# QWERTY6191/projected-lmc

Measured on AMD Instinct MI355X. Metric: MLL+grad iters/sec, n=8192 16-task LMC, higher is better.
Workload: dtype f32; 1 GPU; C3: ProjectedGPModel+ProjectedLMCmll exact training step (PLMC_fast), n=8192 d=8 p=16 q=8 Matern-5/2 fp32; latents sharded q/N per GPU; n_points=8192, n_dim=8, n_tasks=16, n_latents=8, parallelism=latent-shard x1

## Files before the change

### include/plmc.h

```cpp
#ifndef PLMC_H
#define PLMC_H

#include <stddef.h>
#include <stdint.h>

#ifdef __cplusplus
extern "C" {
#endif

enum { PLMC_RBF = 0, PLMC_MATERN12 = 1, PLMC_MATERN32 = 2, PLMC_MATERN52 = 3, PLMC_SPLINE = 4 };

int         plmc_version(void);
int         plmc_block(void);
int64_t     plmc_pad(int64_t n);
int         plmc_max_dim(void);
const char *plmc_last_error(void);
int64_t     plmc_vd_blocks_for(int64_t n_pad, int64_t lda, int elem_bytes);
int64_t     plmc_vd_blocks(int64_t n_pad, int64_t lda);
int64_t     plmc_vd_blocks_keep(int64_t n_pad, int64_t lda);
int64_t     plmc_split_scales_offset(int64_t n_pad, int64_t lda);
int64_t     plmc_grad_scratch_bytes_for(int64_t n_pad, int q, int elem_bytes);
int64_t     plmc_grad_scratch_bytes(int64_t n_pad, int q);
int64_t     plmc_grad_partials_bytes(int64_t n_pad, int q);

// ... 35 lines not shown
int plmc_potrs_aug_f64(double *A, int64_t n_pad, int64_t lda, int naug, int64_t wcol0, int64_t strideA, double *Vd, int q, void *stream);
int plmc_potrs_aug_kept_f32(float *A, int64_t n_pad, int64_t lda, int naug, int64_t wcol0, int64_t strideA, float *Vd, int q,
                            const float *eig_lo, void *stream);
int plmc_potrs_aug_kept_f64(double *A, int64_t n_pad, int64_t lda, int naug, int64_t wcol0, int64_t strideA, double *Vd, int q,
                            const double *eig_lo, void *stream);

int plmc_extract_col_f32(const float *A, int64_t n_pad, int64_t lda, int64_t strideA, int c,
                         float *z, double *quad, int q, void *stream);
int plmc_extract_col_f64(const double *A, int64_t n_pad, int64_t lda, int64_t strideA, int c,
                         double *z, double *quad, int q, void *stream);

int plmc_wt_matvec_f32(const float *W, int64_t n_pad, int64_t ldw, int64_t strideW, const float *z,
                       float *alpha, int q, void *stream);
int plmc_wt_matvec_f64(const double *W, int64_t n_pad, int64_t ldw, int64_t strideW, const double *z,
                       double *alpha, int q, void *stream);

int plmc_gemm_tn_f32(int mode, int M, int N, int K, const float *A, int64_t lda, int64_t strideA, const float *B,
                     int64_t ldb, int64_t strideB, float *C, int64_t ldc, int64_t strideC, int batch, void *stream);
int plmc_gemm_tn_f64(int mode, int M, int N, int K, const double *A, int64_t lda, int64_t strideA, const double *B,
                     int64_t ldb, int64_t strideB, double *C, int64_t ldc, int64_t strideC, int batch, void *stream);
#define PLMC_TRI_A_LOWER 1
#define PLMC_TRI_B_LOWER 2
#define PLMC_TRI_A_UPPER 4
#define PLMC_TRI_C_LOWER 8
#define PLMC_TRI_C_ZERO 16
int plmc_gemm_tn_tri_f32(int mode, int tri, int M, int N, int K, const float *A, int64_t lda, int64_t strideA, const float *B,
                         int64_t ldb, int64_t strideB, float *C, int64_t ldc, int64_t strideC, int batch, void *stream);
int plmc_gemm_tn_tri_f64(int mode, int tri, int M, int N, int K, const double *A, int64_t lda, int64_t strideA, const double *B,
                         int64_t ldb, int64_t strideB, double *C, int64_t ldc, int64_t strideC, int batch, void *stream);

// ... 147 lines not shown
```

### projected-lmc_amd/csrc/potrf.hip

```cpp
#include <stdlib.h>
#include "api_common.hpp"
#include "covariance.hpp"
#include "diag_block.hpp"
#include "bf3_engine.hpp"
#include "chain_engine.hpp"
#include "vd_layout.hpp"
#include "../../include/plmc.h"

namespace plmc {

template <typename T> constexpr int CHAIN_BURST = sizeof(T) == 8 ? 4 : 8;

template <typename T> struct ColMap {
  int u0, nU, Taug, w0, nW;
  int64_t n_pad;
  T *W;
  int64_t ldw, strideW;
};

template <typename T, int NT, bool BURSTED = false>
__global__ __launch_bounds__(NTHREADS, TILE_MIN_WAVES<T>) void k_panel(T *A, int64_t lda, int64_t strideA, int r, ColMap<T> cm,
                                                     const T *__restrict__ Vd, int64_t strideV) {
  __builtin_amdgcn_s_setprio(3);
  __shared__ __align__(16) T smem[tile_smem_elems<T>()];
// ... 596 lines not shown
    for (int u = 0; u < U; ++u)
#pragma unroll
      for (int e = 0; e < EPV; ++e) s[e] += (double)v[u][e] * (double)zz[u];
  }
#pragma unroll
  for (int e = 0; e < EPV; ++e) red[rg][cl + e] = s[e];
  __syncthreads();
  if (threadIdx.x < CW) {
    double t = 0.0;
#pragma unroll
    for (int g = 0; g < NRG; ++g) t += red[g][threadIdx.x];
    alpha[(int64_t)lat * n_pad + colw + threadIdx.x] = (T)t;
  }
}

template <typename T>
__global__ __launch_bounds__(WTMV_NT) void k_w_diag(const T *__restrict__ W, int64_t n_pad, int64_t ldw, int64_t strideW,
                                                    T *__restrict__ kd) {
  using vec_t = typename Traits<T>::vec_t;
  constexpr int EPV = Traits<T>::EPV;
  constexpr int LPR = 128 / EPV;
  constexpr int NRG = WTMV_NT / LPR;
  __shared__ double red[NRG][NB];
  const int lat = blockIdx.y;
  const int cl = (threadIdx.x % LPR) * EPV, rg = threadIdx.x / LPR;
  const int64_t col0 = (int64_t)blockIdx.x * NB;
  const T *Wl = W + (int64_t)lat * strideW + col0 + cl;
  double s[EPV];
#pragma unroll
  for (int e = 0; e < EPV; ++e) s[e] = 0.0;
// ... 23 lines not shown
}

template <typename T, class S>
struct Sweep {
  static constexpr bool bf3 = !std::is_void<S>::value;
  static_assert(!bf3 || sizeof(T) == 4, "split schemes stand in for fp32 products");
  static constexpr double nb = NB, nb3 = nb * nb * nb, esz = sizeof(T);

  T *A;
  int64_t n_pad, lda, strideA, naug_pad, wcol0;
  int q, m, Taug;
  bool with_inverse, keep;
  const float *eig_lo = nullptr;
  double *logdet = nullptr;
  int *info = nullptr;
  T *Vd, *Wg, *Vg2[2], *Ph, *Pbulk;
  unsigned short *Pl[2], *Praw, *VgP2[2], *Wk, *Uk;
  float *scl;
  int64_t strideV, pl_lat, sc_lat, uk_step;
  T *WA;
  const Knobs &kn;
  double hthr;
  unsigned bulk_lds;
  int grp, ng, chain_pool;
  hipStream_t st, C = nullptr, H = nullptr;
  hipEvent_t e_entry = nullptr, e_v = nullptr, e_gh = nullptr, e_p = nullptr, e_hd = nullptr, e_tail = nullptr, e_doneC = nullptr,
             e_doneH = nullptr, e_prev = nullptr, e_sc = nullptr;

  Sweep(T *A_, int64_t n_pad_, int64_t lda_, int naug, int64_t wcol0_, int64_t strideA_, T *Vd_, int q_, bool with_inverse_, bool keep_,
        int grp_, unsigned bulk_lds_, hipStream_t st_)
// ... 168 lines not shown
      if (!WA) return;
      const int g0 = G0(gi), G = G0(gi + 1) - g0;
      hipLaunchKernelGGL((k_wtri_planes<S>), dim3(G * (G + 1) / 2, q), dim3(NTHREADS), 0, s, (const float *)WA, lda, strideA, g0, (const float *)scl,
                         sc_lat, Wk, pl_lat, n_pad);
    }
  }
  void raw_planes0(hipStream_t s, const ColMap<T> &cm) {
    if constexpr (bf3) {
      const int nt = cm.nU + cm.Taug + cm.nW;
      if (nt > 0)
        hipLaunchKernelGGL((k_raw_planes<S>), dim3(nt, G0(1), q), dim3(NTHREADS), 0, s, (const float *)A, lda, strideA, 0, cm, Praw, pl_lat, wcol0,
                           (const float *)scl, sc_lat);
    }
  }

  bool bind_streams() {
    if (!kn.serial) bind_sweep_ctx(st, 8);
    C = kn.serial ? nullptr : side_stream();
    H = kn.serial ? nullptr : (kn.bulk_streams == 1 ? st : side_stream(1));
    hipEvent_t *const ev[] = {&e_entry, &e_v, &e_gh, &e_p, &e_hd, &e_tail, &e_doneC, &e_doneH, &e_prev};
    bool la = C && H && ng > 2;
    for (int i = 0; i < 9; ++i) la = (*ev[i] = sync_event(i)) && la;
    e_sc = sync_event(12);
    return la;
  }

  int inputs(const AssembleJob *job) {
    if (job) {
      const int rc = assemble_rows(*job, (int)sizeof(T), A, lda, strideA, q, 0, m, st);
      if (rc != 0) return rc;
// ... 9 lines not shown
    raw_planes0(st, cm_buf(G0(1), m - G0(1), Taug, 0, 0));
    for (int gi = 0; gi < ng; ++gi) {
      const int g0 = G0(gi), g1 = G0(gi + 1), g2 = G0(gi + 2);
      chain(gi, st);
      vtrans(gi, st);
      wtri_planes(gi, st);
      if (bf3) {
        gpanel(g0, g1 - g0, cm_buf(g1, g2 - g1, 0, 0, 0), gi & 1, st, 1);
        gpanel(g0, g1 - g0, cm_buf(g2, m - g2, Taug, 0, g0), gi & 1, st, 0);
        update(g1, m - g1, g0, g1 - 1, cm_buf(g1, m - g1, Taug, 0, g1), st, PK_TRAIL, g2, g2, false, g2);
        update(g1, g2 - g1, g0, g1 - 1, cm_buf(g1, g2 - g1, 0, 0, 0), st, PK_TRAIL_HEAD, 0, 0, true);
      } else {
        gpanel(g0, g1 - g0, cm_buf(g1, m - g1, Taug, 0, g0), gi & 1, st, 0);
        update(g1, m - g1, g0, g1 - 1, cm_buf(g1, m - g1, Taug, 0, g1), st, PK_TRAIL);
      }
    }
    return finish(st);
  }

  int lookahead(const AssembleJob *job) {
    const bool fused = job && e_sc;
    if (fused) {
      const int rc = assemble_rows(*job, (int)sizeof(T), A, lda, strideA, q, 0, G0(1), st, G0(1));
      if (rc != 0) return rc;
      scan(st, 0, (int64_t)G0(1) * NB, 0, SCAN_PARTS / 2);
    } else {
      const int rc = inputs(job);
      if (rc != 0) return rc;
    }
    (void)hipEventRecord(e_entry, st);
// ... 16 lines not shown
      (void)hipEventRecord(e_v, C);
      if (gi > 0 || bf3) (void)hipStreamWaitEvent(C, e_hd, 0);
      gpanel(g0, G, cm_buf(g1, g2 - g1, 0, 0, 0), gi & 1, C, 1);
      (void)hipEventRecord(e_gh, C);
      if (gi > 0) (void)hipStreamWaitEvent(C, e_tail, 0);
      update(g1, g2 - g1, g0, g1 - 1, cm_buf(g1, g2 - g1, 0, 0, 0), C, PK_TRAIL_HEAD, 0, 0, true);

      (void)hipStreamWaitEvent(H, e_v, 0);
      wtri_planes(gi, H);
      gpanel(g0, G, cm_buf(g2, m - g2, Taug, 0, g0), gi & 1, H, 0);
      (void)hipEventRecord(e_p, H);
      (void)hipStreamWaitEvent(H, e_gh, 0);
      if (gi > 0) (void)hipStreamWaitEvent(H, e_tail, 0);
      update(g1, g2 - g1, g0, g1 - 1, cm_buf(g2, m - g2, Taug, 0, g1), H, PK_TRAIL_HEAD, 0, 0, false, g2);
      (void)hipEventRecord(e_hd, H);

      (void)hipStreamWaitEvent(st, e_p, 0);
      (void)hipStreamWaitEvent(st, e_gh, 0);
      update(g2, m - g2, g0, g1 - 1, cm_buf(g2, m - g2, Taug, 0, g1), st, PK_TRAIL);
      (void)hipEventRecord(e_tail, st);
    }
    const int rc_fin = finish(C);
    (void)hipEventRecord(e_doneC, C);
    (void)hipEventRecord(e_doneH, H);
    (void)hipStreamWaitEvent(st, e_doneC, 0);
    (void)hipStreamWaitEvent(st, e_doneH, 0);
    (void)hipEventRecord(e_prev, st);
    return rc_fin;
  }
};

template <typename T, class S>
int potrf_impl(T *A, int64_t n_pad, int64_t lda, int naug, int64_t strideA, T *Vd, double *logdet, int *info,
               int with_inverse_arg, int q, const float *eig_lo, void *stream, const AssembleJob *job = nullptr) {
  PLMC_REQUIRE((with_inverse_arg & 2) == 0, "with_inverse bit 1 (K^-1 accumulated in the sweep) is gone: use plmc_kinv_grad_* behind the sweep");
  const bool with_inverse = (with_inverse_arg & 1) != 0;
  const bool keep = !std::is_void<S>::value && (with_inverse_arg & 4) != 0 && with_inverse;
  PLMC_REQUIRE(A && Vd && logdet && info, "null pointer");
  PLMC_REQUIRE(n_pad > 0 && n_pad % NB == 0 && lda % NB == 0 && lda >= n_pad, "n_pad/lda must be multiples of NB");
  const int64_t naug_pad = plmc_pad(naug);
  PLMC_REQUIRE(naug >= 0 && n_pad + naug_pad + (with_inverse ? n_pad : 0) <= lda,
               "lda too small for naug (+ the n_pad columns of the inverse factor)");
  PLMC_REQUIRE(q > 0 && aligned16(A) && aligned16(Vd), "bad q or unaligned buffer");
  const Knobs &kn = knobs();
  const int grp = (!keep && kn.grp > 0 && kn.grp < GMAX) ? kn.grp : GMAX;
  const unsigned bulk_lds = (unsigned)(kn.bulk_lds >= 0 ? kn.bulk_lds : (q == 1 ? 20000 : (q == 2 ? 16000 : 0)));
  Sweep<T, S> sw(A, n_pad, lda, naug, n_pad + naug_pad, strideA, Vd, q, with_inverse, keep, grp, bulk_lds, (hipStream_t)stream);
  sw.eig_lo = eig_lo;
  sw.logdet = logdet;
  sw.info = info;
  const double npd = (double)n_pad;
  ProfScope whole(PK_SWEEP, sw.st, q * (with_inverse ? 2.0 : 1.0) * npd * npd * npd / 3.0, 0.0);
  sw.clear();
  return sw.bind_streams() ? sw.lookahead(job) : sw.one_stream(job);
}

bool vd_w_planes(const float *Vd, int64_t n_pad, int64_t lda, const unsigned short **wk, int64_t *wk_lat_stride, const float **w_scale,
                 int64_t *w_scale_lat_stride) {
  const VdLayout L(n_pad, lda, 4, false);
  if (L.wk < 0) return false;
  *wk = L.at<const unsigned short>(Vd, L.wk);
  *wk_lat_stride = L.stride_u16();
  *w_scale = L.at<const float>(Vd, L.scl) + SC_SW;
  *w_scale_lat_stride = L.stride_f32();
  return true;
// ... 85 lines not shown
  PLMC_REQUIRE(n_pad > 0 && n_pad % NB == 0 && q > 0 && aligned16(W), "n_pad must be a multiple of NB");
  ProfScope ps(PK_WTMV, (hipStream_t)stream, q * (double)n_pad * n_pad, q * ((double)n_pad * n_pad / 2) * sizeof(T));
  hipLaunchKernelGGL(k_w_diag<T>, dim3((unsigned)(n_pad / NB), q), dim3(WTMV_NT), 0, (hipStream_t)stream, W, n_pad, ldw, strideW,
                     kinv_diag);
  return launch_status(__func__);
}

}

extern "C" {
int64_t plmc_vd_blocks_for(int64_t n_pad, int64_t lda, int elem_bytes) { return plmc::VdLayout(n_pad, lda, elem_bytes, false).blocks; }
int64_t plmc_vd_blocks(int64_t n_pad, int64_t lda) { return plmc_vd_blocks_for(n_pad, lda, 4); }
int64_t plmc_vd_blocks_keep(int64_t n_pad, int64_t lda) { return plmc::VdLayout(n_pad, lda, 4, true).blocks; }
int64_t plmc_split_scales_offset(int64_t n_pad, int64_t lda) { return plmc::VdLayout(n_pad, lda, 4, false).scl * plmc::NB * plmc::NB; }
static int potrf_f32_any(float *A, int64_t n_pad, int64_t lda, int naug, int64_t strideA, float *Vd, double *logdet, int *info,
                         int with_inverse, int q, const float *eig_lo, void *stream, const plmc::AssembleJob *job = nullptr) {
  const int split = plmc::knobs().split;
  if (split == 0) return plmc::potrf_impl<float, void>(A, n_pad, lda, naug, strideA, Vd, logdet, info, with_inverse, q, nullptr, stream, job);
  if (split == 2 && eig_lo)
    return plmc::potrf_impl<float, plmc::SplitH2>(A, n_pad, lda, naug, strideA, Vd, logdet, info, with_inverse, q, eig_lo, stream, job);
  return plmc::potrf_impl<float, plmc::SplitB3>(A, n_pad, lda, naug, strideA, Vd, logdet, info, with_inverse, q, nullptr, stream, job);
}
int plmc_factorize_ex_f32(int kind, const float *X, int n, int d, const float *ell, const float *oscale, const float *noise, float *A,
                          int64_t n_pad, int64_t lda, int naug, int64_t strideA, float *Vd, double *logdet, int *info, int with_inverse, int q,
                          const float *eig_lo, void *stream) {
  PLMC_REQUIRE(n_pad == plmc_pad(n), "n_pad must be plmc_pad(n)");
  const plmc::AssembleJob job{kind, n, d, X, ell, oscale, noise};
  return potrf_f32_any(A, n_pad, lda, naug, strideA, Vd, logdet, info, with_inverse, q, eig_lo, stream, &job);
}
int plmc_factorize_ex_f64(int kind, const double *X, int n, int d, const double *ell, const double *oscale, const double *noise, double *A,
                          int64_t n_pad, int64_t lda, int naug, int64_t strideA, double *Vd, double *logdet, int *info, int with_inverse, int q,
                          const double *eig_lo, void *stream) {
  (void)eig_lo;
  PLMC_REQUIRE(n_pad == plmc_pad(n), "n_pad must be plmc_pad(n)");
  const plmc::AssembleJob job{kind, n, d, X, ell, oscale, noise};
  return plmc::potrf_impl<double, void>(A, n_pad, lda, naug, strideA, Vd, logdet, info, with_inverse, q, nullptr, stream, &job);
}
// ... 38 lines not shown
  return potrf_f32_any(A, n_pad, lda, naug, strideA, Vd, logdet, info, with_inverse, q, nullptr, stream);
}
int plmc_potrf_f64(double *A, int64_t n_pad, int64_t lda, int naug, int64_t strideA, double *Vd, double *logdet,
                   int *info, int with_inverse, int q, void *stream) {
  return plmc::potrf_impl<double, void>(A, n_pad, lda, naug, strideA, Vd, logdet, info, with_inverse, q, nullptr, stream);
}
int plmc_potrf_ex_f32(float *A, int64_t n_pad, int64_t lda, int naug, int64_t strideA, float *Vd, double *logdet,
                      int *info, int with_inverse, int q, const float *eig_lo, void *stream) {
  return potrf_f32_any(A, n_pad, lda, naug, strideA, Vd, logdet, info, with_inverse, q, eig_lo, stream);
}
int plmc_potrf_ex_f64(double *A, int64_t n_pad, int64_t lda, int naug, int64_t strideA, double *Vd, double *logdet,
                      int *info, int with_inverse, int q, const double *eig_lo, void *stream) {
  (void)eig_lo;
  return plmc::potrf_impl<double, void>(A, n_pad, lda, naug, strideA, Vd, logdet, info, with_inverse, q, nullptr, stream);
}
int plmc_potrs_aug_f32(float *A, int64_t n_pad, int64_t lda, int naug, int64_t wcol0, int64_t strideA, float *Vd, int q, void *stream) {
  return plmc::potrs_aug_at<float>(A, n_pad, lda, naug, wcol0, strideA, Vd, q, stream);
}
int plmc_potrs_aug_f64(double *A, int64_t n_pad, int64_t lda, int naug, int64_t wcol0, int64_t strideA, double *Vd, int q, void *stream) {
  return plmc::potrs_aug_at<double>(A, n_pad, lda, naug, wcol0, strideA, Vd, q, stream);
}
int plmc_potrs_aug_kept_f32(float *A, int64_t n_pad, int64_t lda, int naug, int64_t wcol0, int64_t strideA, float *Vd, int q, const float *eig_lo,
                            void *stream) {
  const int split = plmc::knobs().split;
  if (split == 0) return plmc::potrs_aug_at<float>(A, n_pad, lda, naug, wcol0, strideA, Vd, q, stream);
  if (split == 2 && eig_lo) return plmc::potrs_aug_kept<plmc::SplitH2>(A, n_pad, lda, naug, wcol0, strideA, Vd, q, stream);
  return plmc::potrs_aug_kept<plmc::SplitB3>(A, n_pad, lda, naug, wcol0, strideA, Vd, q, stream);
}
int plmc_potrs_aug_kept_f64(double *A, int64_t n_pad, int64_t lda, int naug, int64_t wcol0, int64_t strideA, double *Vd, int q, const double *eig_lo,
                            void *stream) {
// ... 27 lines not shown
```

### projected-lmc_amd/projectedlmc/_engine.py

```python
import math
import os

import torch

from . import _hip
from . import settings
from ._pivot import PivotCheck, deferred_pivot_checks, walk

LOG2PI = math.log(2.0 * math.pi)


class Workspace:

    def __init__(self, n, q, naug, dtype, device, with_inverse=True, keep_planes=False, ncomp=1, sm=False):
        L = _hip.lib()
        self.n, self.q, self.naug, self.dtype, self.device = n, q, naug, dtype, device
        self.ncomp = ncomp
        self.with_inverse = bool(with_inverse)
        self.keep_planes = bool(keep_planes) and self.with_inverse and dtype == torch.float32
        self.NB = L.cdll.plmc_block()
        self.n_pad = int(L.cdll.plmc_pad(n))
        self.naug_pad = int(L.cdll.plmc_pad(naug)) if naug > 0 else 0
        self.wcol0 = self.n_pad + self.naug_pad
        self.lda = self.wcol0 + (self.n_pad if with_inverse else 0)
# ... 2 lines not shown
        self.strideA = self.n_pad * self.lda
        esz = torch.empty((), dtype=dtype).element_size()
        vd_blocks = L.cdll.plmc_vd_blocks_keep(self.n_pad, self.lda) if self.keep_planes else L.cdll.plmc_vd_blocks_for(self.n_pad, self.lda, esz)
        self.Vd = torch.empty(q, int(vd_blocks), self.NB, self.NB, dtype=dtype, device=device)
        self.m = self.n_pad // self.NB
        self.A = torch.empty(q, self.n_pad, self.lda, dtype=dtype, device=device)
        self.logdet = torch.empty(q, dtype=torch.float64, device=device)
        self.quad = torch.empty(q, dtype=torch.float64, device=device)
        self.info = torch.empty(q, dtype=torch.int32, device=device)
        self.z = torch.empty(q, self.n_pad, dtype=dtype, device=device)
        self.W = self.alpha = self.partials = None
        if with_inverse:
            self.W = self.A[:, :, self.wcol0:self.wcol0 + self.n_pad]
            self.ldw, self.strideW = self.lda, self.strideA
            self.alpha = torch.empty(q, self.n_pad, dtype=dtype, device=device)
            nbytes = int(L.cdll.plmc_sm_grad_partials_bytes(self.n_pad, q, ncomp, esz) if sm
                         else L.cdll.plmc_grad_partials_bytes(self.n_pad, q * ncomp))
            self.partials = torch.empty(nbytes // 8, dtype=torch.float64, device=device)


_ws_cache = {}


def _release(ws):
    pending = getattr(ws, "pending", None)
    if pending is not None:
        torch.cuda.current_stream(ws.device).wait_event(pending)
        ws.pending = None


# ... 31 lines not shown

def free_workspaces():
    _drop_all()


def _contig(t, dtype=None):
    if t is None:
        return None
    t = t.detach()
    if dtype is not None and t.dtype != dtype:
        t = t.to(dtype)
    return t.contiguous()


_SM = {"plmc_assemble": "plmc_assemble_sm", "plmc_assemble_cross": "plmc_assemble_cross_sm",
       "plmc_factorize_ex": "plmc_factorize_sm_ex", "plmc_kinv_grad_vd": "plmc_kinv_grad_sm_vd"}
_ADD = {"plmc_assemble": "plmc_assemble_add", "plmc_assemble_cross": "plmc_assemble_cross_add",
        "plmc_factorize_ex": "plmc_factorize_add_ex", "plmc_kinv_grad_vd": "plmc_kinv_grad_add_vd"}


def is_sm(ell):
    return ell.dim() == 4


def n_components(ell):
    return ell.shape[2] if ell.dim() == 4 else (ell.shape[1] if ell.dim() == 3 else 1)


def kind_code(kind):
    return None if kind == "sm" else _hip.KIND[kind]


def grad_table_width(ell):
# ... 23 lines not shown
            means.record_stream(stream)
        L.call(_SM[base], dt, *head[1:], ell.shape[2], _hip.ptr(scales), _hip.ptr(means), *tail)
    elif ell.dim() == 3:
        L.call(_ADD[base], dt, *head, ell.shape[1], _hip.ptr(ell), *tail)
    else:
        L.call(base, dt, *head, _hip.ptr(ell), *tail)


def _split_grad_table(g, ell_shape, os_shape):
    ne = 1
    for s_ in ell_shape[1:]:
        ne *= s_
    return g[:, :ne].reshape(ell_shape), g[:, ne], (None if os_shape is None else g[:, ne + 1:].reshape(os_shape))


def factorize(kind, X, ell, oscale, noise, rhs, ws, Xs=None):
    L = _hip.lib()
    dt, dev = ws.dtype, ws.device
    st = _hip.stream_ptr(dev)
    k = kind_code(kind)
    q, n, d = ws.q, ws.n, X.shape[1]
    fused = os.environ.get("PLMC_FUSED_ASSEMBLE", "1") != "0"
    if not fused:
        _kernel_call(L, "plmc_assemble", dt, (k, _hip.ptr(X), n, d), ell, (_hip.ptr(oscale), _hip.ptr(noise),
                     _hip.ptr(ws.A), ws.lda, ws.strideA, q, st))
    nrhs = 0 if rhs is None else rhs.shape[1]
    if ws.naug_pad > 0:
        L.call("plmc_write_rhs", dt, _hip.ptr(rhs), nrhs, n, _hip.ptr(ws.A), ws.lda, ws.strideA, 0, ws.naug_pad, q, st)
    if Xs is not None:
        _kernel_call(L, "plmc_assemble_cross", dt, (k, _hip.ptr(X), n, _hip.ptr(Xs), Xs.shape[0], d), ell,
                     (_hip.ptr(oscale), _hip.ptr(ws.A), ws.lda, ws.strideA, ws.n_pad + nrhs, ws.n_pad, q, st))
    flags = (1 | (4 if ws.keep_planes else 0)) if ws.with_inverse else 0
    if fused:
        _kernel_call(L, "plmc_factorize_ex", dt, (k, _hip.ptr(X), n, d), ell, (_hip.ptr(oscale), _hip.ptr(noise), _hip.ptr(ws.A), ws.n_pad,
                     ws.lda, ws.naug, ws.strideA, _hip.ptr(ws.Vd), _hip.ptr(ws.logdet), _hip.ptr(ws.info), flags, q, _hip.ptr(noise), st))
    else:
        L.call("plmc_potrf_ex", dt, _hip.ptr(ws.A), ws.n_pad, ws.lda, ws.naug, ws.strideA, _hip.ptr(ws.Vd),
               _hip.ptr(ws.logdet), _hip.ptr(ws.info), flags, q, _hip.ptr(noise), st)


def factorize_checked(kind, X, ell, oscale, noise, rhs, ws, Xs=None):
    factorize(kind, X, ell, oscale, noise, rhs, ws, Xs)
    if not settings.check_cholesky.on():
        return 0.0
    check = PivotCheck.eager(ws)
    if not check.failed():
        return 0.0

    def attempt(jit):
        factorize(kind, X, ell, oscale, noise + jit, rhs, ws, Xs)
        return PivotCheck.eager(ws), None

    return walk(ws.dtype, check, attempt)[0]


class ExactLatentLogProb(torch.autograd.Function):

    @staticmethod
    def forward(ctx, X, ell, oscale, noise, y, kind, table=None):
        _hip.require_device(X, ell, noise, y)
        L = _hip.lib()
        dt, dev = y.dtype, y.device
        if dt not in (torch.float32, torch.float64):
            raise TypeError("projectedlmc hot path supports float32 and float64 tensors")
        q, n = y.shape
        d = X.shape[1]
        _check_kernel_shape(L, ell)
        G = n_components(ell)
        need_grad = any(ctx.needs_input_grad[1:5]) or table is not None
        Xc, ellc, osc, nzc, yc = (_contig(t, dt) for t in (X, ell, oscale, noise, y))
        ws = get_workspace(n, q, 1, dt, dev, need_grad, G, is_sm(ell))
        st = _hip.stream_ptr(dev)
        grad = table if table is not None else (torch.empty(q, grad_table_width(ell), dtype=torch.float64, device=dev) if need_grad else None)
        check = settings.check_cholesky.on()

        def enqueue(noise_eff):
            factorize(kind, Xc, ellc, osc, noise_eff, yc.reshape(q, 1, n), ws)
            info = PivotCheck(ws) if check else None
            L.call("plmc_extract_col", dt, _hip.ptr(ws.A), ws.n_pad, ws.lda, ws.strideA, 0, _hip.ptr(ws.z),
                   _hip.ptr(ws.quad), q, st)
            if need_grad:
                L.call("plmc_wt_matvec", dt, _hip.ptr(ws.W), ws.n_pad, ws.ldw, ws.strideW, _hip.ptr(ws.z),
                       _hip.ptr(ws.alpha), q, st)
                gs = grad_stream(dev)
                gst = st
                if gs is not None:
                    gs.wait_stream(torch.cuda.current_stream(dev))
                    gst = _hip.stream_handle(gs, dev)
                    for t in (grad, Xc, ellc, osc, noise_eff):
                        if t is not None:
                            t.record_stream(gs)
                _kernel_call(L, "plmc_kinv_grad_vd", dt, (kind_code(kind), _hip.ptr(ws.W), ws.n_pad, ws.ldw, ws.strideW,
                             _hip.ptr(ws.alpha), _hip.ptr(Xc), n, d), ellc, (_hip.ptr(osc), _hip.ptr(grad),
                             None, 0, 0, None, _hip.ptr(ws.partials), q, _hip.ptr(noise_eff), _hip.ptr(ws.Vd), gst), stream=gs)
                if gs is not None:
                    ws.pending = torch.cuda.Event()
                    ws.pending.record(gs)
            lp = -0.5 * (ws.quad + ws.logdet + n * LOG2PI)
# ... 83 lines not shown
    det = lambda t: None if t is None else t.detach()
    lp = ExactLatentLogProb.apply(X, det(ell), det(oscale), det(noise), y, kind, hyper.table)
    return lp + hyper.hz


def exact_loo(kind, X, ell, oscale, noise, y):
    _hip.require_device(X, ell, noise, y)
    L = _hip.lib()
    dt, dev = y.dtype, y.device
    q, n = y.shape
    d = X.shape[1]
    Xc, ellc, osc, nzc, yc = (_contig(t, dt) for t in (X, ell, oscale, noise, y))
    _check_kernel_shape(L, ellc)
    ws = get_workspace(n, q, 1, dt, dev, True, n_components(ellc), is_sm(ellc))
    st = _hip.stream_ptr(dev)
    factorize_checked(kind, Xc, ellc, osc, nzc, yc.reshape(q, 1, n), ws)
    L.call("plmc_extract_col", dt, _hip.ptr(ws.A), ws.n_pad, ws.lda, ws.strideA, 0, _hip.ptr(ws.z),
           _hip.ptr(ws.quad), q, st)
    L.call("plmc_wt_matvec", dt, _hip.ptr(ws.W), ws.n_pad, ws.ldw, ws.strideW, _hip.ptr(ws.z),
           _hip.ptr(ws.alpha), q, st)
    grad = torch.empty(q, grad_table_width(ellc), dtype=torch.float64, device=dev)
    kd = torch.empty(q, ws.n_pad, dtype=dt, device=dev)
    _kernel_call(L, "plmc_kinv_grad_vd", dt, (kind_code(kind), _hip.ptr(ws.W), ws.n_pad, ws.ldw, ws.strideW, _hip.ptr(ws.alpha),
                 _hip.ptr(Xc), n, d), ellc, (_hip.ptr(osc), _hip.ptr(grad), None, 0, 0, _hip.ptr(kd),
                 _hip.ptr(ws.partials), q, _hip.ptr(nzc), _hip.ptr(ws.Vd), st))
    sigma2 = 1.0 / kd[:, :n]
    return sigma2, ws.alpha[:, :n] * sigma2


class PosteriorCache:

    def __init__(self):
        self.key, self.ws = None, None
        self.seen = None
        self.hits = self.misses = 0
# ... 94 lines not shown
```

### projected-lmc_amd/projectedlmc/_hip.py

```python
import ctypes
import os

import torch

_HERE = os.path.dirname(os.path.abspath(__file__))
LIB_PATH = os.environ.get("PLMC_LIB") or os.path.join(_HERE, "libplmc_hip.so")

ABI_VERSION = 4
KIND = {"rbf": 0, "matern12": 1, "matern32": 2, "matern52": 3, "spline": 4}

_c = ctypes
_P = _c.c_void_p
_I = _c.c_int
_L = _c.c_int64

_TYPED = {
    "plmc_assemble": [_I, _P, _I, _I, _P, _P, _P, _P, _L, _L, _I, _P],
    "plmc_assemble_add": [_I, _P, _I, _I, _I, _P, _P, _P, _P, _L, _L, _I, _P],
    "plmc_assemble_sm": [_P, _I, _I, _I, _P, _P, _P, _P, _P, _L, _L, _I, _P],
    "plmc_write_rhs": [_P, _I, _I, _P, _L, _L, _I, _I, _I, _P],
    "plmc_assemble_cross": [_I, _P, _I, _P, _I, _I, _P, _P, _P, _L, _L, _L, _L, _I, _P],
    "plmc_assemble_cross_add": [_I, _P, _I, _P, _I, _I, _I, _P, _P, _P, _L, _L, _L, _L, _I, _P],
    "plmc_assemble_cross_sm": [_P, _I, _P, _I, _I, _I, _P, _P, _P, _P, _L, _L, _L, _L, _I, _P],
    "plmc_potrf": [_P, _L, _L, _I, _L, _P, _P, _P, _I, _I, _P],
    "plmc_potrf_ex": [_P, _L, _L, _I, _L, _P, _P, _P, _I, _I, _P, _P],
    "plmc_factorize_ex": [_I, _P, _I, _I, _P, _P, _P, _P, _L, _L, _I, _L, _P, _P, _P, _I, _I, _P, _P],
    "plmc_factorize_add_ex": [_I, _P, _I, _I, _I, _P, _P, _P, _P, _L, _L, _I, _L, _P, _P, _P, _I, _I, _P, _P],
    "plmc_factorize_sm_ex": [_P, _I, _I, _I, _P, _P, _P, _P, _P, _L, _L, _I, _L, _P, _P, _P, _I, _I, _P, _P],
    "plmc_potrs_aug": [_P, _L, _L, _I, _L, _L, _P, _I, _P],
    "plmc_potrs_aug_kept": [_P, _L, _L, _I, _L, _L, _P, _I, _P, _P],
    "plmc_extract_col": [_P, _L, _L, _L, _I, _P, _P, _I, _P],
    "plmc_wt_matvec": [_P, _L, _L, _L, _P, _P, _I, _P],
    "plmc_w_diag": [_P, _L, _L, _L, _P, _I, _P],
    "plmc_gemm_tn": [_I, _I, _I, _I, _P, _L, _L, _P, _L, _L, _P, _L, _L, _I, _P],
    "plmc_gemm_tn_tri": [_I, _I, _I, _I, _I, _P, _L, _L, _P, _L, _L, _P, _L, _L, _I, _P],
    "plmc_kinv_grad": [_I, _P, _L, _L, _L, _P, _P, _I, _I, _P, _P, _P, _P, _L, _L, _P, _P, _I, _P],
    "plmc_kinv_grad_ex": [_I, _P, _L, _L, _L, _P, _P, _I, _I, _P, _P, _P, _P, _L, _L, _P, _P, _I, _P, _P],
    "plmc_kinv_grad_vd": [_I, _P, _L, _L, _L, _P, _P, _I, _I, _P, _P, _P, _P, _L, _L, _P, _P, _I, _P, _P, _P],
    "plmc_kinv_grad_add_vd": [_I, _P, _L, _L, _L, _P, _P, _I, _I, _I, _P, _P, _P, _P, _L, _L, _P, _P, _I, _P, _P, _P],
    "plmc_kinv_grad_sm_vd": [_P, _L, _L, _L, _P, _P, _I, _I, _I, _P, _P, _P, _P, _P, _L, _L, _P, _P, _I, _P, _P, _P],
    "plmc_lmc_assemble": [_I, _P, _I, _I, _I, _I, _P, _P, _P, _P, _P, _L, _P],
    "plmc_lmc_cross": [_I, _P, _I, _P, _I, _I, _I, _I, _P, _P, _P, _P, _L, _L, _L, _P],
    "plmc_lmc_kinv_grad": [_I, _P, _L, _L, _P, _P, _I, _I, _I, _I, _P, _P, _P, _P, _P, _P],
    "plmc_kernel_vjp": [_I, _P, _I, _P, _I, _I, _P, _P, _P, _L, _L, _P, _P, _P, _I, _P],
    "plmc_qr_small": [_P, _I, _I, _L, _P, _L, _P, _L, _P],
    "plmc_comm_allreduce_sum": [_P, _L, _P],
    "plmc_posterior_moments": [_P, _L, _L, _L, _I, _P, _P, _I, _P],
    "plmc_mix_posterior": [_P, _P, _P, _I, _I, _I, _c.c_double, _P, _P, _P],
}
_PLAIN = {
    "plmc_version": ([], _I),
    "plmc_block": ([], _I),
    "plmc_pad": ([_L], _L),
    "plmc_vd_blocks": ([_L, _L], _L),
    "plmc_vd_blocks_for": ([_L, _L, _I], _L),
    "plmc_vd_blocks_keep": ([_L, _L], _L),
    "plmc_split_scales_offset": ([_L, _L], _L),
    "plmc_max_dim": ([], _I),
    "plmc_max_components": ([], _I),
    "plmc_sm_max_mixtures": ([], _I),
    "plmc_sm_max_dim": ([], _I),
    "plmc_sm_grad_partials_bytes": ([_L, _I, _I, _I], _L),
    "plmc_qr_max": ([], _I),
    "plmc_last_error": ([], _c.c_char_p),
    "plmc_grad_scratch_bytes": ([_L, _I], _L),
    "plmc_grad_scratch_bytes_for": ([_L, _I, _I], _L),
    "plmc_grad_partials_bytes": ([_L, _I], _L),
    "plmc_lmc_grad_len": ([_I, _I, _I], _L),
    "plmc_lmc_grad_scratch_bytes": ([_L, _I, _I, _I], _L),
    "plmc_prof_enable": ([_I], _I),
    "plmc_prof_kernels": ([], _I),
    "plmc_prof_name": ([_I], _c.c_char_p),
# ... 141 lines not shown
```

Measured before the change: 57.36 iters/sec.

## Fuse alpha matvec into Cholesky sweep, computing row blocks as groups finish

Computes z, its squared norm and alpha = W^T z incrementally inside the blocked Cholesky sweep. Each row group is processed once it is final, on the head stream, and partial sums are carried in a new double-precision scratch buffer. This replaces the separate extract_col and wt_matvec launches that ran after factorization, aiming to hide that memory-bound matvec behind the trailing updates. In exchange it adds per-group kernel launches, scratch traffic and extra cross-stream ordering in the sweep.

```diff
diff --git a/include/plmc.h b/include/plmc.h
--- a/include/plmc.h
+++ b/include/plmc.h
@@ -73,6 +73,38 @@
                        float *alpha, int q, void *stream);
 int plmc_wt_matvec_f64(const double *W, int64_t n_pad, int64_t ldw, int64_t strideW, const double *z,
                        double *alpha, int q, void *stream);
+
+int64_t plmc_alpha_scratch_bytes(int64_t n_pad, int q);
+int plmc_potrf_alpha_ex_f32(float *A, int64_t n_pad, int64_t lda, int naug, int64_t strideA, float *Vd, double *logdet, int *info,
+                            int with_inverse, int q, const float *eig_lo, float *alpha, float *z, double *quad, double *alpha_scratch,
+                            void *stream);
+int plmc_potrf_alpha_ex_f64(double *A, int64_t n_pad, int64_t lda, int naug, int64_t strideA, double *Vd, double *logdet, int *info,
+                            int with_inverse, int q, const double *eig_lo, double *alpha, double *z, double *quad, double *alpha_scratch,
+                            void *stream);
+int plmc_factorize_alpha_ex_f32(int kind, const float *X, int n, int d, const float *ell, const float *oscale, const float *noise,
+                                float *A, int64_t n_pad, int64_t lda, int naug, int64_t strideA, float *Vd, double *logdet, int *info,
+                                int with_inverse, int q, const float *eig_lo, float *alpha, float *z, double *quad,
+                                double *alpha_scratch, void *stream);
+int plmc_factorize_alpha_ex_f64(int kind, const double *X, int n, int d, const double *ell, const double *oscale, const double *noise,
+                                double *A, int64_t n_pad, int64_t lda, int naug, int64_t strideA, double *Vd, double *logdet, int *info,
+                                int with_inverse, int q, const double *eig_lo, double *alpha, double *z, double *quad,
+                                double *alpha_scratch, void *stream);
+int plmc_factorize_add_alpha_ex_f32(int kind, const float *X, int n, int d, int ncomp, const float *ell, const float *oscale,
+                                    const float *noise, float *A, int64_t n_pad, int64_t lda, int naug, int64_t strideA, float *Vd,
+                                    double *logdet, int *info, int with_inverse, int q, const float *eig_lo, float *alpha, float *z,
+                                    double *quad, double *alpha_scratch, void *stream);
+int plmc_factorize_add_alpha_ex_f64(int kind, const double *X, int n, int d, int ncomp, const double *ell, const double *oscale,
+                                    const double *noise, double *A, int64_t n_pad, int64_t lda, int naug, int64_t strideA, double *Vd,
+                                    double *logdet, int *info, int with_inverse, int q, const double *eig_lo, double *alpha, double *z,
+                                    double *quad, double *alpha_scratch, void *stream);
+int plmc_factorize_sm_alpha_ex_f32(const float *X, int n, int d, int nmix, const float *scales, const float *means,
+                                   const float *weights, const float *noise, float *A, int64_t n_pad, int64_t lda, int naug,
+                                   int64_t strideA, float *Vd, double *logdet, int *info, int with_inverse, int q, const float *eig_lo,
+                                   float *alpha, float *z, double *quad, double *alpha_scratch, void *stream);
+int plmc_factorize_sm_alpha_ex_f64(const double *X, int n, int d, int nmix, const double *scales, const double *means,
+                                   const double *weights, const double *noise, double *A, int64_t n_pad, int64_t lda, int naug,
+                                   int64_t strideA, double *Vd, double *logdet, int *info, int with_inverse, int q, const double *eig_lo,
+                                   double *alpha, double *z, double *quad, double *alpha_scratch, void *stream);
 
 int plmc_gemm_tn_f32(int mode, int M, int N, int K, const float *A, int64_t lda, int64_t strideA, const float *B,
                      int64_t ldb, int64_t strideB, float *C, int64_t ldc, int64_t strideC, int batch, void *stream);
diff --git a/projected-lmc_amd/csrc/potrf.hip b/projected-lmc_amd/csrc/potrf.hip
--- a/projected-lmc_amd/csrc/potrf.hip
+++ b/projected-lmc_amd/csrc/potrf.hip
@@ -634,6 +634,100 @@
   }
 }
 
+constexpr int ALPHA_NRG = 32;
+__host__ __device__ inline int64_t alpha_scratch_lat(int64_t n_pad) { return (int64_t)ALPHA_NRG * n_pad + NTHREADS; }
+template <typename T>
+struct AlphaOut {
+  T *alpha = nullptr, *z = nullptr;
+  double *quad = nullptr, *scratch = nullptr;
+  explicit operator bool() const { return alpha != nullptr; }
+};
+
+template <typename T, int CW = NB>
+__global__ __launch_bounds__(WTMV_NT * CW / NB) void k_wt_matvec_rows(const T *__restrict__ W, int64_t n_pad, int64_t ldw, int64_t strideW,
+                                                                      const T *__restrict__ Az, int64_t lda, int64_t strideA, int64_t r0,
+                                                                      int64_t r1, int last, T *__restrict__ z, T *__restrict__ alpha,
+                                                                      double *__restrict__ quad, double *__restrict__ scratch) {
+  using vec_t = typename Traits<T>::vec_t;
+  constexpr int EPV = Traits<T>::EPV;
+  constexpr int LPR = CW / EPV;
+  constexpr int NRG = WTMV_NT / (NB / EPV);
+  constexpr int NT = WTMV_NT * CW / NB;
+  static_assert(NRG <= ALPHA_NRG && NT >= NTHREADS && NB % NRG == 0, "scratch layout");
+  __shared__ double red[NRG][CW];
+  __shared__ T zs[GMAX * NB];
+  const int lat = blockIdx.y;
+  const int cl = (threadIdx.x % LPR) * EPV, rg = threadIdx.x / LPR;
+  const int64_t colw = (int64_t)blockIdx.x * CW;
+  const int64_t col0 = colw / NB * NB;
+  const int64_t lo = r0 > col0 ? r0 : col0;
+  const int nz = (int)(r1 - lo);
+  const T *Azl = Az + (int64_t)lat * strideA;
+  double *sl = scratch + (int64_t)lat * alpha_scratch_lat(n_pad);
+  for (int i = threadIdx.x; i < nz; i += NT) zs[i] = Azl[(lo + i) * lda];
+  __syncthreads();
+  if (blockIdx.x == 0) {
+    double *rq = &red[0][0];
+    for (int i = threadIdx.x; i < nz; i += NT) z[(int64_t)lat * n_pad + r0 + i] = zs[i];
+    if (threadIdx.x < NTHREADS) {
+      double *qp = sl + (int64_t)ALPHA_NRG * n_pad;
+      double s = r0 == 0 ? 0.0 : qp[threadIdx.x];
+      const int first = (int)(((int64_t)threadIdx.x - r0 % NTHREADS + NTHREADS) % NTHREADS);
+      for (int i = first; i < nz; i += NTHREADS) {
+        T v = zs[i];
+        s += (double)v * (double)v;
+      }
+      if (!last) qp[threadIdx.x] = s;
+      else rq[threadIdx.x] = s;
+    }
+    if (last) {
+      __syncthreads();
+      for (int o = NTHREADS / 2; o > 0; o >>= 1) {
+        if (threadIdx.x < o) rq[threadIdx.x] += rq[threadIdx.x + o];
+        __syncthreads();
+      }
+      if (threadIdx.x == 0) quad[lat] = rq[0];
+      __syncthreads();
+    }
+  }
+  const T *Wl = W + (int64_t)lat * strideW + colw + cl;
+  double *cp = sl + (int64_t)rg * n_pad + colw + cl;
+  double s[EPV];
+#pragma unroll
+  for (int e = 0; e < EPV; ++e) s[e] = r0 > col0 ? cp[e] : 0.0;
+  constexpr int U = CW == NB ? 4 : 8;
+  for (int64_t l = lo + rg; l < r1; l += U * NRG) {
+    vec_t v[U];
+    T zz[U];
+#pragma unroll
+    for (int u = 0; u < U; ++u) {
+      const int64_t ll = l + u * NRG;
+      const int64_t lc = ll < r1 ? ll : r1 - 1;
+      v[u] = *reinterpret_cast<const vec_t *>(Wl + lc * ldw);
+      const T zv = zs[lc - lo];
+      zz[u] = ll < r1 ? zv : T(0);
+    }
+#pragma unroll
+    for (int u = 0; u < U; ++u)
+#pragma unroll
+      for (int e = 0; e < EPV; ++e) s[e] += (double)v[u][e] * (double)zz[u];
+  }
+  if (!last) {
+#pragma unroll
+    for (int e = 0; e < EPV; ++e) cp[e] = s[e];
+    return;
+  }
+#pragma unroll
+  for (int e = 0; e < EPV; ++e) red[rg][cl + e] = s[e];
+  __syncthreads();
+  if (threadIdx.x < CW) {
+    double t = 0.0;
+#pragma unroll
+    for (int g = 0; g < NRG; ++g) t += red[g][threadIdx.x];
+    alpha[(int64_t)lat * n_pad + colw + threadIdx.x] = (T)t;
+  }
+}
+
 template <typename T>
 __global__ __launch_bounds__(WTMV_NT) void k_w_diag(const T *__restrict__ W, int64_t n_pad, int64_t ldw, int64_t strideW,
                                                     T *__restrict__ kd) {
@@ -687,6 +781,7 @@
   const float *eig_lo = nullptr;
   double *logdet = nullptr;
   int *info = nullptr;
+  AlphaOut<T> ao;
   T *Vd, *Wg, *Vg2[2], *Ph, *Pbulk;
   unsigned short *Pl[2], *Praw, *VgP2[2], *Wk, *Uk;
   float *scl;
@@ -885,6 +980,19 @@
     }
   }
 
+  void alpha_rows(int gi, hipStream_t s) {
+    if (!ao) return;
+    const int64_t r0 = (int64_t)G0(gi) * NB, r1 = (int64_t)G0(gi + 1) * NB;
+    const int last = gi + 1 >= ng;
+    ProfScope ps(PK_WTMV, s, q * (double)(r1 - r0) * (r0 + r1), q * ((double)(r1 - r0) * (r0 + r1) / 2) * esz);
+#define PLMC_AROWS(CW)                                                                                                              \
+  hipLaunchKernelGGL((k_wt_matvec_rows<T, CW>), dim3((unsigned)(r1 / CW), q), dim3(WTMV_NT * CW / NB), 0, s, (const T *)WA, n_pad, lda, \
+                     strideA, (const T *)(A + n_pad), lda, strideA, r0, r1, last, ao.z, ao.alpha, ao.quad, ao.scratch)
+    if ((int64_t)q * (r1 / NB) < 128) PLMC_AROWS(32);
+    else PLMC_AROWS(NB);
+#undef PLMC_AROWS
+  }
+
   bool bind_streams() {
     if (!kn.serial) bind_sweep_ctx(st, 8);
     C = kn.serial ? nullptr : side_stream();
@@ -924,6 +1032,7 @@
         gpanel(g0, g1 - g0, cm_buf(g1, m - g1, Taug, 0, g0), gi & 1, st, 0);
         update(g1, m - g1, g0, g1 - 1, cm_buf(g1, m - g1, Taug, 0, g1), st, PK_TRAIL);
       }
+      alpha_rows(gi, st);
     }
     return finish(st);
   }
@@ -970,6 +1079,7 @@
       if (gi > 0) (void)hipStreamWaitEvent(H, e_tail, 0);
       update(g1, g2 - g1, g0, g1 - 1, cm_buf(g2, m - g2, Taug, 0, g1), H, PK_TRAIL_HEAD, 0, 0, false, g2);
       (void)hipEventRecord(e_hd, H);
+      if (gi + 1 < ng) alpha_rows(gi, H);
 
       (void)hipStreamWaitEvent(st, e_p, 0);
       (void)hipStreamWaitEvent(st, e_gh, 0);
@@ -979,8 +1089,9 @@
     const int rc_fin = finish(C);
     (void)hipEventRecord(e_doneC, C);
     (void)hipEventRecord(e_doneH, H);
+    (void)hipStreamWaitEvent(st, e_doneH, 0);
+    alpha_rows(ng - 1, st);
     (void)hipStreamWaitEvent(st, e_doneC, 0);
-    (void)hipStreamWaitEvent(st, e_doneH, 0);
     (void)hipEventRecord(e_prev, st);
     return rc_fin;
   }
@@ -988,7 +1099,8 @@
 
 template <typename T, class S>
 int potrf_impl(T *A, int64_t n_pad, int64_t lda, int naug, int64_t strideA, T *Vd, double *logdet, int *info,
-               int with_inverse_arg, int q, const float *eig_lo, void *stream, const AssembleJob *job = nullptr) {
+               int with_inverse_arg, int q, const float *eig_lo, void *stream, const AssembleJob *job = nullptr,
+               const AlphaOut<T> &ao = AlphaOut<T>()) {
   PLMC_REQUIRE((with_inverse_arg & 2) == 0, "with_inverse bit 1 (K^-1 accumulated in the sweep) is gone: use plmc_kinv_grad_* behind the sweep");
   const bool with_inverse = (with_inverse_arg & 1) != 0;
   const bool keep = !std::is_void<S>::value && (with_inverse_arg & 4) != 0 && with_inverse;
@@ -998,6 +1110,10 @@
   PLMC_REQUIRE(naug >= 0 && n_pad + naug_pad + (with_inverse ? n_pad : 0) <= lda,
                "lda too small for naug (+ the n_pad columns of the inverse factor)");
   PLMC_REQUIRE(q > 0 && aligned16(A) && aligned16(Vd), "bad q or unaligned buffer");
+  if (ao.alpha || ao.z || ao.quad || ao.scratch) {
+    PLMC_REQUIRE(ao.alpha && ao.z && ao.quad && ao.scratch, "alpha block: alpha, z, quad and scratch go together");
+    PLMC_REQUIRE(with_inverse && naug >= 1, "alpha block: needs the inverse factor and an augmented column");
+  }
   const Knobs &kn = knobs();
   const int grp = (!keep && kn.grp > 0 && kn.grp < GMAX) ? kn.grp : GMAX;
   const unsigned bulk_lds = (unsigned)(kn.bulk_lds >= 0 ? kn.bulk_lds : (q == 1 ? 20000 : (q == 2 ? 16000 : 0)));
@@ -1005,6 +1121,7 @@
   sw.eig_lo = eig_lo;
   sw.logdet = logdet;
   sw.info = info;
+  sw.ao = ao;
   const double npd = (double)n_pad;
   ProfScope whole(PK_SWEEP, sw.st, q * (with_inverse ? 2.0 : 1.0) * npd * npd * npd / 3.0, 0.0);
   sw.clear();
@@ -1120,13 +1237,25 @@
 int64_t plmc_vd_blocks_keep(int64_t n_pad, int64_t lda) { return plmc::VdLayout(n_pad, lda, 4, true).blocks; }
 int64_t plmc_split_scales_offset(int64_t n_pad, int64_t lda) { return plmc::VdLayout(n_pad, lda, 4, false).scl * plmc::NB * plmc::NB; }
 static int potrf_f32_any(float *A, int64_t n_pad, int64_t lda, int naug, int64_t strideA, float *Vd, double *logdet, int *info,
-                         int with_inverse, int q, const float *eig_lo, void *stream, const plmc::AssembleJob *job = nullptr) {
+                         int with_inverse, int q, const float *eig_lo, void *stream, const plmc::AssembleJob *job = nullptr,
+                         const plmc::AlphaOut<float> &ao = plmc::AlphaOut<float>()) {
   const int split = plmc::knobs().split;
-  if (split == 0) return plmc::potrf_impl<float, void>(A, n_pad, lda, naug, strideA, Vd, logdet, info, with_inverse, q, nullptr, stream, job);
+  if (split == 0) return plmc::potrf_impl<float, void>(A, n_pad, lda, naug, strideA, Vd, logdet, info, with_inverse, q, nullptr, stream, job, ao);
   if (split == 2 && eig_lo)
-    return plmc::potrf_impl<float, plmc::SplitH2>(A, n_pad, lda, naug, strideA, Vd, logdet, info, with_inverse, q, eig_lo, stream, job);
-  return plmc::potrf_impl<float, plmc::SplitB3>(A, n_pad, lda, naug, strideA, Vd, logdet, info, with_inverse, q, nullptr, stream, job);
-}
+    return plmc::potrf_impl<float, plmc::SplitH2>(A, n_pad, lda, naug, strideA, Vd, logdet, info, with_inverse, q, eig_lo, stream, job, ao);
+  return plmc::potrf_impl<float, plmc::SplitB3>(A, n_pad, lda, naug, strideA, Vd, logdet, info, with_inverse, q, nullptr, stream, job, ao);
+}
+static plmc::AlphaOut<float> alpha_out(float *alpha, float *z, double *quad, double *scratch) {
+  plmc::AlphaOut<float> ao;
+  ao.alpha = alpha; ao.z = z; ao.quad = quad; ao.scratch = scratch;
+  return ao;
+}
+static plmc::AlphaOut<double> alpha_out(double *alpha, double *z, double *quad, double *scratch) {
+  plmc::AlphaOut<double> ao;
+  ao.alpha = alpha; ao.z = z; ao.quad = quad; ao.scratch = scratch;
+  return ao;
+}
+int64_t plmc_alpha_scratch_bytes(int64_t n_pad, int q) { return (int64_t)q * plmc::alpha_scratch_lat(n_pad) * (int64_t)sizeof(double); }
 int plmc_factorize_ex_f32(int kind, const float *X, int n, int d, const float *ell, const float *oscale, const float *noise, float *A,
                           int64_t n_pad, int64_t lda, int naug, int64_t strideA, float *Vd, double *logdet, int *info, int with_inverse, int q,
                           const float *eig_lo, void *stream) {
@@ -1195,6 +1324,72 @@
   (void)eig_lo;
   return plmc::potrf_impl<double, void>(A, n_pad, lda, naug, strideA, Vd, logdet, info, with_inverse, q, nullptr, stream);
 }
+#define PLMC_ALPHA_ARGS(T) T *alpha, T *z, double *quad, double *alpha_scratch
+int plmc_potrf_alpha_ex_f32(float *A, int64_t n_pad, int64_t lda, int naug, int64_t strideA, float *Vd, double *logdet, int *info,
+                            int with_inverse, int q, const float *eig_lo, PLMC_ALPHA_ARGS(float), void *stream) {
+  return potrf_f32_any(A, n_pad, lda, naug, strideA, Vd, logdet, info, with_inverse, q, eig_lo, stream, nullptr, alpha_out(alpha, z, quad, alpha_scratch));
+}
+int plmc_potrf_alpha_ex_f64(double *A, int64_t n_pad, int64_t lda, int naug, int64_t strideA, double *Vd, double *logdet, int *info,
+                            int with_inverse, int q, const double *eig_lo, PLMC_ALPHA_ARGS(double), void *stream) {
+  (void)eig_lo;
+  return plmc::potrf_impl<double, void>(A, n_pad, lda, naug, strideA, Vd, logdet, info, with_inverse, q, nullptr, stream, nullptr,
+                                        alpha_out(alpha, z, quad, alpha_scratch));
+}
+int plmc_factorize_alpha_ex_f32(int kind, const float *X, int n, int d, const float *ell, const float *oscale, const float *noise, float *A,
+                                int64_t n_pad, int64_t lda, int naug, int64_t strideA, float *Vd, double *logdet, int *info, int with_inverse,
+                                int q, const float *eig_lo, PLMC_ALPHA_ARGS(float), void *stream) {
+  PLMC_REQUIRE(n_pad == plmc_pad(n), "n_pad must be plmc_pad(n)");
+  const plmc::AssembleJob job{kind, n, d, X, ell, oscale, noise};
+  return potrf_f32_any(A, n_pad, lda, naug, strideA, Vd, logdet, info, with_inverse, q, eig_lo, stream, &job, alpha_out(alpha, z, quad, alpha_scratch));
+}
+int plmc_factorize_alpha_ex_f64(int kind, const double *X, int n, int d, const double *ell, const double *oscale, const double *noise, double *A,
+                                int64_t n_pad, int64_t lda, int naug, int64_t strideA, double *Vd, double *logdet, int *info, int with_inverse,
+                                int q, const double *eig_lo, PLMC_ALPHA_ARGS(double), void *stream) {
+  (void)eig_lo;
+  PLMC_REQUIRE(n_pad == plmc_pad(n), "n_pad must be plmc_pad(n)");
+  const plmc::AssembleJob job{kind, n, d, X, ell, oscale, noise};
+  return plmc::potrf_impl<double, void>(A, n_pad, lda, naug, strideA, Vd, logdet, info, with_inverse, q, nullptr, stream, &job,
+                                        alpha_out(alpha, z, quad, alpha_scratch));
+}
+int plmc_factorize_add_alpha_ex_f32(int kind, const float *X, int n, int d, int ncomp, const float *ell, const float *oscale, const float *noise,
+                                    float *A, int64_t n_pad, int64_t lda, int naug, int64_t strideA, float *Vd, double *logdet, int *info,
+                                    int with_inverse, int q, const float *eig_lo, PLMC_ALPHA_ARGS(float), void *stream) {
+  PLMC_REQUIRE(n_pad == plmc_pad(n), "n_pad must be plmc_pad(n)");
+  PLMC_REQUIRE(kind >= 0 && kind <= plmc::K_MATERN52, "additive kernels take the stationary kinds only (no spline kernel)");
+  PLMC_REQUIRE(ncomp >= 1 && ncomp <= plmc::MAX_COMP, "need 1 <= components <= plmc_max_components()");
+  const plmc::AssembleJob job{kind, n, d, X, ell, oscale, noise, ncomp};
+  return potrf_f32_any(A, n_pad, lda, naug, strideA, Vd, logdet, info, with_inverse, q, eig_lo, stream, &job, alpha_out(alpha, z, quad, alpha_scratch));
+}
+int plmc_factorize_add_alpha_ex_f64(int kind, const double *X, int n, int d, int ncomp, const double *ell, const double *oscale, const double *noise,
+                                    double *A, int64_t n_pad, int64_t lda, int naug, int64_t strideA, double *Vd, double *logdet, int *info,
+                                    int with_inverse, int q, const double *eig_lo, PLMC_ALPHA_ARGS(double), void *stream) {
+  (void)eig_lo;
+  PLMC_REQUIRE(n_pad == plmc_pad(n), "n_pad must be plmc_pad(n)");
+  PLMC_REQUIRE(kind >= 0 && kind <= plmc::K_MATERN52, "additive kernels take the stationary kinds only (no spline kernel)");
+  PLMC_REQUIRE(ncomp >= 1 && ncomp <= plmc::MAX_COMP, "need 1 <= components <= plmc_max_components()");
+  const plmc::AssembleJob job{kind, n, d, X, ell, oscale, noise, ncomp};
+  return plmc::potrf_impl<double, void>(A, n_pad, lda, naug, strideA, Vd, logdet, info, with_inverse, q, nullptr, stream, &job,
+                                        alpha_out(alpha, z, quad, alpha_scratch));
+}
+int plmc_factorize_sm_alpha_ex_f32(const float *X, int n, int d, int nmix, const float *scales, const float *means, const float *weights,
+                                   const float *noise, float *A, int64_t n_pad, int64_t lda, int naug, int64_t strideA, float *Vd, double *logdet,
+                                   int *info, int with_inverse, int q, const float *eig_lo, PLMC_ALPHA_ARGS(float), void *stream) {
+  PLMC_REQUIRE(n_pad == plmc_pad(n), "n_pad must be plmc_pad(n)");
+  PLMC_REQUIRE_SM(nmix, d, means);
+  const plmc::AssembleJob job{0, n, d, X, scales, weights, noise, nmix, means};
+  return potrf_f32_any(A, n_pad, lda, naug, strideA, Vd, logdet, info, with_inverse, q, eig_lo, stream, &job, alpha_out(alpha, z, quad, alpha_scratch));
+}
+int plmc_factorize_sm_alpha_ex_f64(const double *X, int n, int d, int nmix, const double *scales, const double *means, const double *weights,
+                                   const double *noise, double *A, int64_t n_pad, int64_t lda, int naug, int64_t strideA, double *Vd, double *logdet,
+                                   int *info, int with_inverse, int q, const double *eig_lo, PLMC_ALPHA_ARGS(double), void *stream) {
+  (void)eig_lo;
+  PLMC_REQUIRE(n_pad == plmc_pad(n), "n_pad must be plmc_pad(n)");
+  PLMC_REQUIRE_SM(nmix, d, means);
+  const plmc::AssembleJob job{0, n, d, X, scales, weights, noise, nmix, means};
+  return plmc::potrf_impl<double, void>(A, n_pad, lda, naug, strideA, Vd, logdet, info, with_inverse, q, nullptr, stream, &job,
+                                        alpha_out(alpha, z, quad, alpha_scratch));
+}
+#undef PLMC_ALPHA_ARGS
 int plmc_potrs_aug_f32(float *A, int64_t n_pad, int64_t lda, int naug, int64_t wcol0, int64_t strideA, float *Vd, int q, void *stream) {
   return plmc::potrs_aug_at<float>(A, n_pad, lda, naug, wcol0, strideA, Vd, q, stream);
 }
diff --git a/projected-lmc_amd/projectedlmc/_engine.py b/projected-lmc_amd/projectedlmc/_engine.py
--- a/projected-lmc_amd/projectedlmc/_engine.py
+++ b/projected-lmc_amd/projectedlmc/_engine.py
@@ -40,6 +40,7 @@
             self.W = self.A[:, :, self.wcol0:self.wcol0 + self.n_pad]
             self.ldw, self.strideW = self.lda, self.strideA
             self.alpha = torch.empty(q, self.n_pad, dtype=dtype, device=device)
+            self.alpha_scratch = torch.empty(int(L.cdll.plmc_alpha_scratch_bytes(self.n_pad, q)) // 8, dtype=torch.float64, device=device)
             nbytes = int(L.cdll.plmc_sm_grad_partials_bytes(self.n_pad, q, ncomp, esz) if sm
                          else L.cdll.plmc_grad_partials_bytes(self.n_pad, q * ncomp))
             self.partials = torch.empty(nbytes // 8, dtype=torch.float64, device=device)
@@ -101,9 +102,11 @@
 
 
 _SM = {"plmc_assemble": "plmc_assemble_sm", "plmc_assemble_cross": "plmc_assemble_cross_sm",
-       "plmc_factorize_ex": "plmc_factorize_sm_ex", "plmc_kinv_grad_vd": "plmc_kinv_grad_sm_vd"}
+       "plmc_factorize_ex": "plmc_factorize_sm_ex", "plmc_factorize_alpha_ex": "plmc_factorize_sm_alpha_ex",
+       "plmc_kinv_grad_vd": "plmc_kinv_grad_sm_vd"}
 _ADD = {"plmc_assemble": "plmc_assemble_add", "plmc_assemble_cross": "plmc_assemble_cross_add",
-        "plmc_factorize_ex": "plmc_factorize_add_ex", "plmc_kinv_grad_vd": "plmc_kinv_grad_add_vd"}
+        "plmc_factorize_ex": "plmc_factorize_add_ex", "plmc_factorize_alpha_ex": "plmc_factorize_add_alpha_ex",
+        "plmc_kinv_grad_vd": "plmc_kinv_grad_add_vd"}
 
 
 def is_sm(ell):
@@ -157,7 +160,7 @@
     return g[:, :ne].reshape(ell_shape), g[:, ne], (None if os_shape is None else g[:, ne + 1:].reshape(os_shape))
 
 
-def factorize(kind, X, ell, oscale, noise, rhs, ws, Xs=None):
+def factorize(kind, X, ell, oscale, noise, rhs, ws, Xs=None, alpha=False):
     L = _hip.lib()
     dt, dev = ws.dtype, ws.device
     st = _hip.stream_ptr(dev)
@@ -174,16 +177,19 @@
         _kernel_call(L, "plmc_assemble_cross", dt, (k, _hip.ptr(X), n, _hip.ptr(Xs), Xs.shape[0], d), ell,
                      (_hip.ptr(oscale), _hip.ptr(ws.A), ws.lda, ws.strideA, ws.n_pad + nrhs, ws.n_pad, q, st))
     flags = (1 | (4 if ws.keep_planes else 0)) if ws.with_inverse else 0
+    sfx, ablock = "_ex", ()
+    if alpha:
+        sfx, ablock = "_alpha_ex", (_hip.ptr(ws.alpha), _hip.ptr(ws.z), _hip.ptr(ws.quad), _hip.ptr(ws.alpha_scratch))
     if fused:
-        _kernel_call(L, "plmc_factorize_ex", dt, (k, _hip.ptr(X), n, d), ell, (_hip.ptr(oscale), _hip.ptr(noise), _hip.ptr(ws.A), ws.n_pad,
-                     ws.lda, ws.naug, ws.strideA, _hip.ptr(ws.Vd), _hip.ptr(ws.logdet), _hip.ptr(ws.info), flags, q, _hip.ptr(noise), st))
+        _kernel_call(L, "plmc_factorize" + sfx, dt, (k, _hip.ptr(X), n, d), ell, (_hip.ptr(oscale), _hip.ptr(noise), _hip.ptr(ws.A), ws.n_pad,
+                     ws.lda, ws.naug, ws.strideA, _hip.ptr(ws.Vd), _hip.ptr(ws.logdet), _hip.ptr(ws.info), flags, q, _hip.ptr(noise)) + ablock + (st,))
     else:
-        L.call("plmc_potrf_ex", dt, _hip.ptr(ws.A), ws.n_pad, ws.lda, ws.naug, ws.strideA, _hip.ptr(ws.Vd),
-               _hip.ptr(ws.logdet), _hip.ptr(ws.info), flags, q, _hip.ptr(noise), st)
-
-
-def factorize_checked(kind, X, ell, oscale, noise, rhs, ws, Xs=None):
-    factorize(kind, X, ell, oscale, noise, rhs, ws, Xs)
+        L.call("plmc_potrf" + sfx, dt, _hip.ptr(ws.A), ws.n_pad, ws.lda, ws.naug, ws.strideA, _hip.ptr(ws.Vd),
+               _hip.ptr(ws.logdet), _hip.ptr(ws.info), flags, q, _hip.ptr(noise), *ablock, st)
+
+
+def factorize_checked(kind, X, ell, oscale, noise, rhs, ws, Xs=None, alpha=False):
+    factorize(kind, X, ell, oscale, noise, rhs, ws, Xs, alpha)
     if not settings.check_cholesky.on():
         return 0.0
     check = PivotCheck.eager(ws)
@@ -191,7 +197,7 @@
         return 0.0
 
     def attempt(jit):
-        factorize(kind, X, ell, oscale, noise + jit, rhs, ws, Xs)
+        factorize(kind, X, ell, oscale, noise + jit, rhs, ws, Xs, alpha)
         return PivotCheck.eager(ws), None
 
     return walk(ws.dtype, check, attempt)[0]
@@ -218,13 +224,12 @@
         check = settings.check_cholesky.on()
 
         def enqueue(noise_eff):
-            factorize(kind, Xc, ellc, osc, noise_eff, yc.reshape(q, 1, n), ws)
+            factorize(kind, Xc, ellc, osc, noise_eff, yc.reshape(q, 1, n), ws, alpha=need_grad)
             info = PivotCheck(ws) if check else None
-            L.call("plmc_extract_col", dt, _hip.ptr(ws.A), ws.n_pad, ws.lda, ws.strideA, 0, _hip.ptr(ws.z),
-                   _hip.ptr(ws.quad), q, st)
-            if need_grad:
-                L.call("plmc_wt_matvec", dt, _hip.ptr(ws.W), ws.n_pad, ws.ldw, ws.strideW, _hip.ptr(ws.z),
-                       _hip.ptr(ws.alpha), q, st)
+            if not need_grad:
+                L.call("plmc_extract_col", dt, _hip.ptr(ws.A), ws.n_pad, ws.lda, ws.strideA, 0, _hip.ptr(ws.z),
+                       _hip.ptr(ws.quad), q, st)
+            else:
                 gs = grad_stream(dev)
                 gst = st
                 if gs is not None:
@@ -338,11 +343,7 @@
     _check_kernel_shape(L, ellc)
     ws = get_workspace(n, q, 1, dt, dev, True, n_components(ellc), is_sm(ellc))
     st = _hip.stream_ptr(dev)
-    factorize_checked(kind, Xc, ellc, osc, nzc, yc.reshape(q, 1, n), ws)
-    L.call("plmc_extract_col", dt, _hip.ptr(ws.A), ws.n_pad, ws.lda, ws.strideA, 0, _hip.ptr(ws.z),
-           _hip.ptr(ws.quad), q, st)
-    L.call("plmc_wt_matvec", dt, _hip.ptr(ws.W), ws.n_pad, ws.ldw, ws.strideW, _hip.ptr(ws.z),
-           _hip.ptr(ws.alpha), q, st)
+    factorize_checked(kind, Xc, ellc, osc, nzc, yc.reshape(q, 1, n), ws, alpha=True)
     grad = torch.empty(q, grad_table_width(ellc), dtype=torch.float64, device=dev)
     kd = torch.empty(q, ws.n_pad, dtype=dt, device=dev)
     _kernel_call(L, "plmc_kinv_grad_vd", dt, (kind_code(kind), _hip.ptr(ws.W), ws.n_pad, ws.ldw, ws.strideW, _hip.ptr(ws.alpha),
diff --git a/projected-lmc_amd/projectedlmc/_hip.py b/projected-lmc_amd/projectedlmc/_hip.py
--- a/projected-lmc_amd/projectedlmc/_hip.py
+++ b/projected-lmc_amd/projectedlmc/_hip.py
@@ -27,6 +27,10 @@
     "plmc_factorize_ex": [_I, _P, _I, _I, _P, _P, _P, _P, _L, _L, _I, _L, _P, _P, _P, _I, _I, _P, _P],
     "plmc_factorize_add_ex": [_I, _P, _I, _I, _I, _P, _P, _P, _P, _L, _L, _I, _L, _P, _P, _P, _I, _I, _P, _P],
     "plmc_factorize_sm_ex": [_P, _I, _I, _I, _P, _P, _P, _P, _P, _L, _L, _I, _L, _P, _P, _P, _I, _I, _P, _P],
+    "plmc_potrf_alpha_ex": [_P, _L, _L, _I, _L, _P, _P, _P, _I, _I, _P, _P, _P, _P, _P, _P],
+    "plmc_factorize_alpha_ex": [_I, _P, _I, _I, _P, _P, _P, _P, _L, _L, _I, _L, _P, _P, _P, _I, _I, _P, _P, _P, _P, _P, _P],
+    "plmc_factorize_add_alpha_ex": [_I, _P, _I, _I, _I, _P, _P, _P, _P, _L, _L, _I, _L, _P, _P, _P, _I, _I, _P, _P, _P, _P, _P, _P],
+    "plmc_factorize_sm_alpha_ex": [_P, _I, _I, _I, _P, _P, _P, _P, _P, _L, _L, _I, _L, _P, _P, _P, _I, _I, _P, _P, _P, _P, _P, _P],
     "plmc_potrs_aug": [_P, _L, _L, _I, _L, _L, _P, _I, _P],
     "plmc_potrs_aug_kept": [_P, _L, _L, _I, _L, _L, _P, _I, _P, _P],
     "plmc_extract_col": [_P, _L, _L, _L, _I, _P, _P, _I, _P],
@@ -56,6 +60,7 @@
     "plmc_vd_blocks_for": ([_L, _L, _I], _L),
     "plmc_vd_blocks_keep": ([_L, _L], _L),
     "plmc_split_scales_offset": ([_L, _L], _L),
+    "plmc_alpha_scratch_bytes": ([_L, _I], _L),
     "plmc_max_dim": ([], _I),
     "plmc_max_components": ([], _I),
     "plmc_sm_max_mixtures": ([], _I),
```

Result: no change. 57.63 iters/sec, median of 6 (+0.5%).
